# jskvrna/MonoSOWA

Hardware: AMD Instinct MI355X
Metric: MonoDETR training img/s (KITTI 1280x384) (higher is better)
Workload: dtype f32; 1 GPU; MonoDETR resnet50 KITTI 1280x384, fwd+criterion+bwd+AdamW step, per-GPU batch 16, synthetic images + random pseudo-labels; global_batch=16, per_gpu_batch=16, parallelism=dp1, accumulation_micro_steps=1, mixed_cameras=False, queries=550, tuned=True

## Files before the change

monosowa_amd/build.py:

```python
import os
import shutil
import subprocess
import sys

HERE = os.path.dirname(os.path.abspath(__file__))
CSRC = os.path.join(HERE, "csrc")
LIBDIR = os.path.join(HERE, "lib")
ARCH = "gfx950"

LIBS = {
    "libmonosowa_msda.so": ("msda_capi.hip", []),
    "libmonosowa_pointwise.so": ("pointwise.hip", []),
    "libmonosowa_attn.so": ("flash_attn.hip", []),
    "libmonosowa_kitti.so": ("rotate_iou.hip", []),
    "libmonosowa_gemm.so": ("gemm_lt.cpp", ["-lhipblaslt"]),
    "libmonosowa_image.so": ("image_prep.hip", ["-ffp-contract=off"]),
    "libmonosowa_fit.so": ("template_fit.hip", []),
    "libmonosowa_lift.so": ("object_lift.hip", []),
    "libmonosowa_track.so": ("object_track.hip", []),
}

FLAGS = ["-O3", "--offload-arch=" + ARCH, "-munsafe-fp-atomics", "-fPIC", "-shared", "-std=c++17",
         "-fno-gpu-rdc", "-Wall"]


def hipcc():
    exe = shutil.which("hipcc") or "/opt/rocm/bin/hipcc"
    if not os.path.exists(exe):
        raise RuntimeError("hipcc not found: the MI355X-native kernels cannot be built")
    return exe


def source_hash(extra=()):
    import hashlib
    h = hashlib.sha256()
    inc = os.path.normpath(os.path.join(HERE, "..", "include"))
    files = [os.path.join(CSRC, f) for f in os.listdir(CSRC)] + [os.path.join(inc, f) for f in os.listdir(inc)]
    for path in sorted(files):
        if os.path.isfile(path):
            h.update(os.path.basename(path).encode() + b"\0")
            with open(path, "rb") as f:
                h.update(f.read())
            h.update(b"\0")
    for x in extra:
        h.update(str(x).encode() + b"\0")
    return h.hexdigest()


def _recorded_hash(out):
    try:
        with open(out + ".srchash") as f:
            return f.read().strip()
    except OSError:
        return None


def _build_one(out, cmd, want, force, verbose):
    name = os.path.basename(out)
    if not force and os.path.exists(out) and _recorded_hash(out) == want:
        if verbose:
            print("%s: up to date (source hash %s)" % (name, want[:16]), flush=True)
        return False
    if verbose:
        print(" ".join(cmd), flush=True)
    subprocess.check_call(cmd)
    with open(out + ".srchash", "w") as f:
        f.write(want + "\n")
    if verbose:
        print("%s: compiled (source hash %s)" % (name, want[:16]), flush=True)
    return True


def build_host_libs(force=False, verbose=False):
    out = os.path.join(LIBDIR, "libmonosowa_lsap.so")
    src = os.path.join(CSRC, "lsap.cpp")
    flags = ["-O3", "-fPIC", "-shared", "-std=c++17", "-Wall", "-pthread"]
    cmd = [shutil.which("g++") or "g++"] + flags + ["-o", out, src]
    _build_one(out, cmd, source_hash(["g++"] + flags), force, verbose)
    return [out]


def build_all(force=False, verbose=False):
    os.makedirs(LIBDIR, exist_ok=True)
    built = build_host_libs(force, verbose)
    for name, (tu, extra) in LIBS.items():
        out = os.path.join(LIBDIR, name)
        want = source_hash(["hipcc"] + FLAGS + extra)
        _build_one(out, [hipcc()] + FLAGS + ["-o", out, os.path.join(CSRC, tu)] + extra, want, force, verbose)
        built.append(out)
    _stamp_commit()
    return built


def _stamp_commit():
    try:
        root = os.path.dirname(HERE)
        h = subprocess.run(["git", "-C", root, "rev-parse", "--short", "HEAD"], capture_output=True, text=True, timeout=10)
        if h.returncode != 0:
            return
        d = subprocess.run(["git", "-C", root, "status", "--porcelain", "--untracked-files=no"], capture_output=True, text=True, timeout=10)
        with open(os.path.join(LIBDIR, "BUILD_COMMIT"), "w") as f:
            f.write(h.stdout.strip() + ("-dirty" if d.stdout.strip() else "") + "\n")
    except Exception:
        pass


if __name__ == "__main__":
    for p in build_all(force="--force" in sys.argv, verbose=True):
        print("built", p)
```

monosowa_amd/monodetr/backbone.py:

```python
import os

import torch
import torch.nn.functional as F
from torch import nn

from ..pointwise import (affine_relu, affine_relu_supported, bias_act, bias_act_fork, bias_relu_maxpool,
                         bias_relu_maxpool_supported, conv1x1_head, conv1x1_head_supported, conv1x1_tail,
                         conv1x1_tail_ds, conv1x1_tail_ds_supported, conv1x1_tail_supported)
from .misc import NestedTensor
from .position_encoding import build_position_encoding


AFFINE_IN_KERNEL = True
CACHE_SCALE_SHIFT = True


class FrozenBatchNorm2d(nn.Module):

    def __init__(self, n, eps=1e-5):
        super().__init__()
        self.register_buffer("weight", torch.ones(n))
        self.register_buffer("bias", torch.zeros(n))
        self.register_buffer("running_mean", torch.zeros(n))
        self.register_buffer("running_var", torch.ones(n))
        self.eps = eps

    def _load_from_state_dict(self, state_dict, prefix, local_metadata, strict, missing_keys,
                              unexpected_keys, error_msgs):
        state_dict.pop(prefix + "num_batches_tracked", None)
        super()._load_from_state_dict(state_dict, prefix, local_metadata, strict, missing_keys,
                                      unexpected_keys, error_msgs)

    def scale_shift(self):
        bufs = (self.weight, self.bias, self.running_mean, self.running_var)
        key = tuple((b.data_ptr(), b._version, b.device, b.dtype) for b in bufs)
        cached = self.__dict__.get("_scale_shift")
        if CACHE_SCALE_SHIFT and cached is not None and cached[0] == key:
            return cached[1], cached[2]
        scale = self.weight * (self.running_var + self.eps).rsqrt()
        shift = self.bias - self.running_mean * scale
        self.__dict__["_scale_shift"] = (key, scale, shift)
        return scale, shift

    def forward(self, x):
        scale, shift = self.scale_shift()
        return x * scale.reshape(1, -1, 1, 1) + shift.reshape(1, -1, 1, 1)


_PARAM_EPOCH = [0]


def _bump_param_epoch(*_args, **_kwargs):
    _PARAM_EPOCH[0] += 1


try:
    from torch.optim.optimizer import register_optimizer_step_post_hook
    register_optimizer_step_post_hook(_bump_param_epoch)
except ImportError:
    _PARAM_EPOCH = None


def folded_weight(conv, bn, scale):
    w = conv.weight
    if (w.requires_grad and torch.is_grad_enabled()) or _PARAM_EPOCH is None:
        return w * scale.view(-1, 1, 1, 1)
    key = (w.data_ptr(), w._version, scale.data_ptr(), scale._version, _PARAM_EPOCH[0] if w.requires_grad else -1)
    cached = conv.__dict__.get("_folded")
    if cached is None or cached[0] != key:
        with torch.no_grad():
            cached = conv.__dict__["_folded"] = (key, (w * scale.view(-1, 1, 1, 1)).contiguous(memory_format=torch.channels_last)
                                                 if w.is_contiguous(memory_format=torch.channels_last) else w * scale.view(-1, 1, 1, 1))
    return cached[1]


def _summed_shift(bn, other):
    a, b = bn.scale_shift()[1], other.scale_shift()[1]
    key = (a.data_ptr(), a._version, b.data_ptr(), b._version)
    cached = bn.__dict__.get("_summed_shift")
    if cached is None or cached[0] != key:
        with torch.no_grad():
            cached = bn.__dict__["_summed_shift"] = (key, a + b)
    return cached[1]


CONV1X1_EPILOGUE = int(os.environ.get("MONOSOWA_CONV1X1_EPILOGUE", "3"))
CONV1X1_SCALED_GRAD = 1


def _pixels(t):
    return t.permute(0, 2, 3, 1).reshape(-1, t.shape[1])


class _Conv1x1BnAct(torch.autograd.Function):

    @staticmethod
    def forward(ctx, x, w, scale, shift, residual, n_out):
        from .. import gemm_lt
        N, C, H, W = x.shape
        K = w.shape[0]
        y = torch.empty((N, K, H, W), dtype=torch.float32, device=x.device, memory_format=torch.channels_last)
        gemm_lt.gemm_nt(_pixels(x), w.reshape(K, C), scale, shift, None if residual is None else _pixels(residual), True, out=_pixels(y))
        ctx.save_for_backward(x, w, scale, y)
        ctx.has_res = residual is not None
        return (y,) + tuple(y.detach() for _ in range(n_out - 1))

    @staticmethod
    def backward(ctx, *grads):
        from .. import gemm_lt
        from ..pointwise import relu_grad_from_output
        x, w, scale, y = ctx.saved_tensors
        N, C, H, W = x.shape
        K = w.shape[0]
        given = [t for t in grads if t is not None]
        pre_scaled = bool(CONV1X1_SCALED_GRAD) and not ctx.has_res and len(given) == 1 and scale.data_ptr() % 16 == 0 and scale.is_contiguous()
        g = relu_grad_from_output(given, y, scale if pre_scaled else None)
        gx = gw = None
        w2 = w.reshape(K, C)
        if ctx.needs_input_grad[0]:
            ws = w2 if pre_scaled else w2 * scale.view(-1, 1)
            if CONV1X1_EPILOGUE & 2:
                gx = torch.empty_like(x)
                gemm_lt.gemm_nn(_pixels(g), ws, out=_pixels(gx))
            else:
                gx = torch.ops.aten.convolution_backward(g, x, ws.view(K, C, 1, 1), None, (1, 1), (0, 0), (1, 1), False, (0, 0), 1,
                                                         (True, False, False))[0]
        if ctx.needs_input_grad[1]:
            gw = torch.ops.aten.convolution_backward(g, x, w, None, (1, 1), (0, 0), (1, 1), False, (0, 0), 1, (False, True, False))[1]
            if not pre_scaled:
                gw = gw * scale.view(-1, 1, 1, 1)
        return gx, gw, None, None, (g if ctx.has_res else None), None


def conv1x1_no_grad(x, conv, scale, shift, residual, relu):
    if not (CONV1X1_EPILOGUE & 1) or conv.kernel_size != (1, 1) or conv.stride != (1, 1) or conv.groups != 1 or conv.padding != (0, 0) \
            or not x.is_cuda or x.dim() != 4 or x.dtype != torch.float32 or not x.is_contiguous(memory_format=torch.channels_last) \
            or x.shape[1] % 4 or conv.weight.shape[0] % 4 \
            or (torch.is_grad_enabled() and (x.requires_grad or conv.weight.requires_grad or (residual is not None and residual.requires_grad))) \
            or (residual is not None and not (residual.shape[1] == conv.weight.shape[0] and residual.dtype == torch.float32
                                              and residual.is_contiguous(memory_format=torch.channels_last))):
        return None
    from .. import gemm_lt
    N, C, H, W = x.shape
    K = conv.weight.shape[0]
    y = torch.empty((N, K, H, W), dtype=torch.float32, device=x.device, memory_format=torch.channels_last)
    with torch.no_grad():
        gemm_lt.gemm_nt(_pixels(x), conv.weight.reshape(K, C), scale, shift, None if residual is None else _pixels(residual), relu, out=_pixels(y))
    return y


def conv1x1_epilogue_applies(x, conv, residual=None):
    from .. import gemm_lt
    return bool(CONV1X1_EPILOGUE & 1) and conv.kernel_size == (1, 1) and conv.stride == (1, 1) and conv.groups == 1 and conv.padding == (0, 0) \
        and x.is_cuda and x.dim() == 4 and x.dtype == torch.float32 and torch.is_grad_enabled() and conv.weight.requires_grad \
        and x.is_contiguous(memory_format=torch.channels_last) and x.shape[1] % 4 == 0 and conv.weight.shape[0] % 4 == 0 \
        and (residual is None or (residual.shape[1] == conv.weight.shape[0] and residual.is_contiguous(memory_format=torch.channels_last)
                                  and residual.dtype == torch.float32))


def conv_bn_fork(x, conv, bn, residual, n_out=2, residual_bn=None):
    if isinstance(bn, FrozenBatchNorm2d):
        scale, shift = bn.scale_shift()
        if residual_bn is not None:
            shift = _summed_shift(bn, residual_bn)
        if conv1x1_epilogue_applies(x, conv, residual):
            return _Conv1x1BnAct.apply(x, conv.weight, scale, shift, residual, n_out)
        y = conv1x1_no_grad(x, conv, scale, shift, residual, True)
        if y is not None:
            return (y,) * n_out
        y = F.conv2d(x, folded_weight(conv, bn, scale), None, conv.stride, conv.padding, conv.dilation, conv.groups)
        return bias_act_fork(y, shift, residual, n_out)
    assert residual_bn is None
    out = conv_bn(x, conv, bn, residual)
    return (out,) * n_out


def conv_bn(x, conv, bn, residual=None, relu=True):
    if isinstance(bn, FrozenBatchNorm2d):
        scale, shift = bn.scale_shift()
        if relu and residual is None and conv1x1_epilogue_applies(x, conv):
            return _Conv1x1BnAct.apply(x, conv.weight, scale, shift, None, 1)[0]
        if AFFINE_IN_KERNEL and relu and residual is None and conv.weight.requires_grad and torch.is_grad_enabled() and x.is_cuda:
            y = F.conv2d(x, conv.weight, None, conv.stride, conv.padding, conv.dilation, conv.groups)
            if affine_relu_supported(y, scale):
                return affine_relu(y, scale, shift)
            return torch.relu(y * scale.view(1, -1, 1, 1) + shift.view(1, -1, 1, 1))
        y = conv1x1_no_grad(x, conv, scale, shift, residual, relu)
        if y is not None:
            return y
        y = F.conv2d(x, folded_weight(conv, bn, scale), None, conv.stride, conv.padding, conv.dilation, conv.groups)
        return bias_act(y, shift, residual, relu)
    y = bn(conv(x))
    if residual is not None:
        y = y + residual
    return F.relu(y, inplace=True) if relu else y


FOLD_DOWNSAMPLE_SHIFT = os.environ.get("MONOSOWA_FOLD_DS_SHIFT", "1") != "0"
FUSED_FROZEN_DS = os.environ.get("MONOSOWA_FUSED_FROZEN_DS", "1") != "0"
FUSED_FROZEN_TAIL = os.environ.get("MONOSOWA_FUSED_FROZEN_TAIL", "1") != "0"
FUSED_STEM = os.environ.get("MONOSOWA_FUSED_STEM", "1") != "0"


def stem(x, conv, bn):
    if isinstance(bn, FrozenBatchNorm2d):
        scale, shift = bn.scale_shift()
        w = folded_weight(conv, bn, scale)
        if not (w.requires_grad and torch.is_grad_enabled()):
            y = F.conv2d(x, w, None, conv.stride, conv.padding, conv.dilation, conv.groups)
            if FUSED_STEM and bias_relu_maxpool_supported(y, shift):
                return bias_relu_maxpool(y, shift)
            return F.max_pool2d(bias_act(y, shift, None, True), kernel_size=3, stride=2, padding=1)
    return F.max_pool2d(conv_bn(x, conv, bn), kernel_size=3, stride=2, padding=1)


class Bottleneck(nn.Module):
    expansion = 4

    def __init__(self, inplanes, planes, stride=1, downsample=None, dilation=1, norm_layer=FrozenBatchNorm2d):
        super().__init__()
        self.conv1 = nn.Conv2d(inplanes, planes, 1, bias=False)
        self.bn1 = norm_layer(planes)
        self.conv2 = nn.Conv2d(planes, planes, 3, stride=stride, padding=dilation, dilation=dilation, bias=False)
        self.bn2 = norm_layer(planes)
        self.conv3 = nn.Conv2d(planes, planes * self.expansion, 1, bias=False)
        self.bn3 = norm_layer(planes * self.expansion)
        self.downsample = downsample

    def forward(self, x):
        xa, xb = x if isinstance(x, tuple) else (x, x)
        n_out = getattr(self, "n_out", 2)
        whole = self._frozen_block(xa, xb, n_out) if FUSED_FROZEN_TAIL else None
        if whole is not None:
            return whole
        out = conv_bn(xa, self.conv1, self.bn1)
        out = conv_bn(out, self.conv2, self.bn2)
        if self.downsample is None:
            return conv_bn_fork(out, self.conv3, self.bn3, xb, n_out)
        ds_conv, ds_bn = self.downsample[0], self.downsample[1]
        if FOLD_DOWNSAMPLE_SHIFT and isinstance(ds_bn, FrozenBatchNorm2d) and isinstance(self.bn3, FrozenBatchNorm2d):
            identity = F.conv2d(xb, folded_weight(ds_conv, ds_bn, ds_bn.scale_shift()[0]), None, ds_conv.stride, ds_conv.padding,
                                ds_conv.dilation, ds_conv.groups)
            return conv_bn_fork(out, self.conv3, self.bn3, identity, n_out, residual_bn=ds_bn)
        identity = conv_bn(xb, ds_conv, ds_bn, relu=False)
        return conv_bn_fork(out, self.conv3, self.bn3, identity, n_out)


    def _frozen_block(self, xa, xb, n_out):
        bn1, bn2, bn3, ds = self.bn1, self.bn2, self.bn3, self.downsample
        if self.conv3.weight.shape[:2] != (256, 64) or not xa.is_cuda or not isinstance(bn2, FrozenBatchNorm2d) \
                or not isinstance(bn3, FrozenBatchNorm2d) or (ds is not None and not isinstance(ds[1], FrozenBatchNorm2d)):
            return None
        if torch.is_grad_enabled() and (xa.requires_grad or xb.requires_grad or self.conv1.weight.requires_grad
                                        or self.conv2.weight.requires_grad or self.conv3.weight.requires_grad
                                        or (ds is not None and ds[0].weight.requires_grad)):
            return None
        h1 = None
        conv1 = self.conv1
        if isinstance(bn1, FrozenBatchNorm2d) and conv1.kernel_size == (1, 1) and conv1.stride == (1, 1) and conv1.weight.shape[0] == 64:
            scale1, shift1 = bn1.scale_shift()
            w1 = folded_weight(conv1, bn1, scale1)
            cached = self.__dict__.get("_head_w")
            if cached is None or cached[0] is not w1:
                with torch.no_grad():
                    cached = self.__dict__["_head_w"] = (w1, w1.reshape(64, -1).t().contiguous())
            if conv1x1_head_supported(xa, cached[1]):
                h1 = conv1x1_head(xa, cached[1], shift1)
        if h1 is None:
            h1 = conv_bn(xa, conv1, bn1)
        (scale2, shift2), (scale3, shift3) = bn2.scale_shift(), bn3.scale_shift()
        w3 = folded_weight(self.conv3, bn3, scale3)
        cached = self.__dict__.get("_tail_w")
        if cached is None or cached[0] is not w3:
            with torch.no_grad():
                cached = self.__dict__["_tail_w"] = (w3, w3.reshape(256, 64).t().contiguous())
        w_kn = cached[1]
        conv2 = self.conv2
        raw2 = F.conv2d(h1, folded_weight(conv2, bn2, scale2), None, conv2.stride, conv2.padding, conv2.dilation, conv2.groups)
        if ds is not None and FUSED_FROZEN_DS and ds[0].kernel_size == (1, 1) and ds[0].stride == (1, 1) and ds[0].weight.shape[:2] == (256, 64):
            wd = folded_weight(ds[0], ds[1], ds[1].scale_shift()[0])
            cached_d = self.__dict__.get("_tail_wd")
            if cached_d is None or cached_d[0] is not wd:
                with torch.no_grad():
                    cached_d = self.__dict__["_tail_wd"] = (wd, wd.reshape(256, 64).t().contiguous())
            if conv1x1_tail_ds_supported(raw2, w_kn, xb, cached_d[1]):
                return (conv1x1_tail_ds(raw2, shift2, w_kn, xb, cached_d[1], _summed_shift(bn3, ds[1])),) * n_out
        if ds is None:
            identity, b_out = xb, shift3
        else:
            identity = F.conv2d(xb, folded_weight(ds[0], ds[1], ds[1].scale_shift()[0]), None, ds[0].stride, ds[0].padding,
                                ds[0].dilation, ds[0].groups)
            b_out = _summed_shift(bn3, ds[1])
        if not conv1x1_tail_supported(raw2, w_kn, identity):
            out = bias_act(raw2, shift2, None, True)
            y = F.conv2d(out, w3, None, self.conv3.stride, self.conv3.padding, self.conv3.dilation, self.conv3.groups)
            return (bias_act(y, b_out, identity, True),) * n_out
        return (conv1x1_tail(raw2, shift2, w_kn, b_out, identity),) * n_out


_DEPTHS = {"resnet50": (3, 4, 6, 3), "resnet101": (3, 4, 23, 3)}


class ResNetBody(nn.Module):

    def __init__(self, name, dilation=False, norm_layer=FrozenBatchNorm2d, return_interm_layers=True):
        super().__init__()
        if name not in _DEPTHS:
            raise ValueError("backbone %r is not supported (resnet50 / resnet101)" % name)
        self.inplanes, self._dil = 64, 1
        self.conv1 = nn.Conv2d(3, 64, 7, stride=2, padding=3, bias=False)
        self.bn1 = norm_layer(64)
        self.layer1 = self._make_layer(64, _DEPTHS[name][0], 1, False, norm_layer)
        self.layer2 = self._make_layer(128, _DEPTHS[name][1], 2, False, norm_layer)
        self.layer3 = self._make_layer(256, _DEPTHS[name][2], 2, False, norm_layer)
        self.layer4 = self._make_layer(512, _DEPTHS[name][3], 2, dilation, norm_layer)
        self.return_interm_layers = return_interm_layers
        for m in self.modules():
            if isinstance(m, nn.Conv2d):
                nn.init.kaiming_normal_(m.weight, mode="fan_out", nonlinearity="relu")

    def _make_layer(self, planes, blocks, stride, dilate, norm_layer):
        prev_dil = self._dil
        if dilate:
            self._dil *= stride
            stride = 1
        downsample = None
        if stride != 1 or self.inplanes != planes * 4:
            downsample = nn.Sequential(nn.Conv2d(self.inplanes, planes * 4, 1, stride=stride, bias=False),
                                       norm_layer(planes * 4))
        layers = [Bottleneck(self.inplanes, planes, stride, downsample, prev_dil, norm_layer)]
        self.inplanes = planes * 4
        layers += [Bottleneck(self.inplanes, planes, dilation=self._dil, norm_layer=norm_layer) for _ in range(1, blocks)]
        return nn.Sequential(*layers)

    def forward(self, x):
        x = stem(x, self.conv1, self.bn1)
        x = self.layer1(x)
        if self.return_interm_layers:
            self.layer2[-1].n_out = self.layer3[-1].n_out = 3
        c3 = self.layer2(x)
        c4 = self.layer3(c3[:2])
        c5 = self.layer4(c4[:2])
        out5 = c5[0]
        if c5[1] is not c5[0]:
            out5.fork_twin = c5[1]
        return {"0": c3[-1], "1": c4[-1], "2": out5} if self.return_interm_layers else {"0": out5}


class Backbone(nn.Module):

    def __init__(self, name, train_backbone, return_interm_layers, dilation, depth=False, pretrained=False):
        super().__init__()
        if depth:
            raise NotImplementedError("4-channel (RGB-D) input is off in every shipped config (model.depth: False)")
        if pretrained:
            raise RuntimeError("model.pretrained: True needs torchvision's ImageNet download, which is not "
                               "available offline; load a state dict instead and set pretrained: False")
        assert name not in ("resnet18", "resnet34"), "number of channels are hard coded"
        self.body = ResNetBody(name, dilation, FrozenBatchNorm2d, return_interm_layers)
        for pname, p in self.body.named_parameters():
            if not train_backbone or ("layer2" not in pname and "layer3" not in pname and "layer4" not in pname):
                p.requires_grad_(False)
        if return_interm_layers:
            self.strides, self.num_channels = [8, 16, 32], [512, 1024, 2048]
        else:
            self.strides, self.num_channels = [32], [2048]
        if dilation:
            self.strides[-1] = self.strides[-1] // 2

    def forward(self, images):
        out = {}
        for name, x in self.body(images).items():
            mask = torch.zeros(x.shape[0], x.shape[2], x.shape[3], dtype=torch.bool, device=x.device)
            out[name] = NestedTensor(x, mask, all_valid=True)
        return out


class Joiner(nn.Sequential):
    def __init__(self, backbone, position_embedding):
        super().__init__(backbone, position_embedding)
        self.strides = backbone.strides
        self.num_channels = backbone.num_channels

    def forward(self, images):
        xs = self[0](images)
        out = [x for _, x in sorted(xs.items())]
        pos = [self[1](x).to(x.tensors.dtype) for x in out]
# ... 10 lines not shown
```

monosowa_amd/pointwise.py:

```python
import ctypes
import os

import numpy as np
import torch

from . import flops
from ._lib import raw_stream, on_device, DeterministicSwitch, alert_not_deterministic

_PATH = os.path.join(os.path.dirname(os.path.abspath(__file__)), "lib", "libmonosowa_pointwise.so")
SYMBOLS = ("mono_bias_act_f32", "mono_bias_relu_maxpool_nhwc_f32", "mono_conv1x1_tail_f32", "mono_conv1x1_tail_ds_f32", "mono_conv1x1_head_f32", "mono_relu_grad_f32", "mono_relu_grad2_f32", "mono_relu_grad3_f32", "mono_bias_relu_mask_f32", "mono_relu_grad_mask_f32", "mono_affine_relu_mask_f32", "mono_affine_relu_grad_f32", "mono_dropout_add_layernorm_fwd_f32",
           "mono_dropout_add_layernorm_bwd_f32", "mono_groupnorm_nhwc_fwd_f32", "mono_groupnorm_nhwc_bwd_f32", "mono_groupnorm_blocks", "mono_colsum_f32", "mono_colsum_strided_f32", "mono_reduce_blocks", "mono_adamw_step_f32", "mono_adamw_step_guarded_f32", "mono_grad_guard_f32", "mono_relu_dropout_fwd_f32",
           "mono_relu_dropout_bwd_f32", "mono_matched_losses_fwd_f32", "mono_matched_losses_bwd_f32", "mono_ddn_loss_blocks",
           "mono_ddn_loss_fwd_f32", "mono_ddn_loss_bwd_f32", "mono_depth_expect_fwd_f32", "mono_depth_expect_bwd_f32", "mono_focal_fwd_f32", "mono_focal_bwd_f32", "mono_head_tail_fwd_f32", "mono_head_tail_bwd_f32", "mono_match_cost_f32", "mono_refine_reference_f32", "mono_relu_dropout_bwd_colsum_f32", "mono_sum_slices_f32", "mono_colsum_any_blocks", "mono_colsum_any_f32", "mono_relu_grad_mask3_f32", "mono_lsap_match_flat_f32",
           "mono_linear_wgrad_workspace", "mono_linear_wgrad_f32", "mono_colsum_levels_blocks", "mono_colsum_levels_f32", "mono_relu_grad_scale_f32",
           "mono_set_deterministic", "mono_groupnorm_stats_doubles", "mono_groupnorm_part_doubles", "mono_grad_accumulate_f32", "mono_ema_update_f32", "mono_step_stats_f32",
           "mono_label_audit_f32", "mono_matched_losses_weighted_fwd_f32", "mono_matched_losses_weighted_bwd_f32", "mono_focal_weighted_fwd_f32",
           "mono_focal_weighted_bwd_f32", "mono_ddn_loss_weighted_fwd_f32", "mono_ddn_loss_weighted_bwd_f32", "mono_focal_weighted_max_cells",
           "mono_ignore_flags_f32", "mono_focal_ignore_fwd_f32", "mono_focal_ignore_bwd_f32", "mono_focal_weighted_ignore_fwd_f32",
           "mono_focal_weighted_ignore_bwd_f32", "mono_ddn_loss_ignore_fwd_f32", "mono_ddn_loss_ignore_bwd_f32",
           "mono_ddn_loss_weighted_ignore_fwd_f32", "mono_ddn_loss_weighted_ignore_bwd_f32")
_lib = None


def load():
# ... 136 lines not shown
        lib.mono_ddn_loss_weighted_fwd_f32.restype = I
        lib.mono_ddn_loss_weighted_fwd_f32.argtypes = [P] * 6 + [I] * 5 + [LL] * 3 + [F] * 6 + [P]
        lib.mono_ddn_loss_weighted_bwd_f32.restype = I
        lib.mono_ddn_loss_weighted_bwd_f32.argtypes = [P] * 7 + [I] * 5 + [LL] * 3 + [F] * 6 + [P]
        for name, n_ptr in (("mono_ddn_loss_ignore_fwd_f32", 8), ("mono_ddn_loss_ignore_bwd_f32", 8), ("mono_ddn_loss_weighted_ignore_fwd_f32", 9),
                            ("mono_ddn_loss_weighted_ignore_bwd_f32", 9)):
            getattr(lib, name).restype = I
            getattr(lib, name).argtypes = [P] * n_ptr + [I] * 6 + [LL] * 3 + [F] * 6 + [P]
        _lib = lib
    return _lib


def _nhwc_ok(t):
    return t.is_cuda and t.dtype == torch.float32 and t.dim() == 4 and t.size(1) % 4 == 0 \
        and t.is_contiguous(memory_format=torch.channels_last) and t.data_ptr() % 16 == 0


USE_RELU_MASK = True


class _BiasAct(torch.autograd.Function):
    @staticmethod
    def forward(ctx, y, bias, residual, relu):
        rows = y.numel() // y.size(1)
        res_ptr = residual.data_ptr() if residual is not None else None
        mask = None
        with on_device(y.device):
            st = raw_stream()
            if relu and USE_RELU_MASK and (y.requires_grad or (residual is not None and residual.requires_grad)):
                mask = torch.empty(y.numel() // 4, dtype=torch.uint8, device=y.device)
                code = load().mono_bias_relu_mask_f32(y.data_ptr(), bias.data_ptr(), res_ptr, mask.data_ptr(), rows, y.size(1), st)
            else:
                code = load().mono_bias_act_f32(y.data_ptr(), bias.data_ptr(), res_ptr, rows, y.size(1), int(relu), st)
        if code:
            raise RuntimeError("mono_bias_act_f32 failed with code %d" % code)
        ctx.mark_dirty(y)
        ctx.relu = relu
        ctx.has_res = residual is not None
        ctx.bias_grad = bias.requires_grad
        ctx.masked = mask is not None
        if relu:
            ctx.save_for_backward(mask if mask is not None else y)
        return y

    @staticmethod
    def backward(ctx, grad):
        if ctx.relu:
            (y,) = ctx.saved_tensors
            grad = grad.contiguous(memory_format=torch.channels_last)
            g = torch.empty_like(grad, memory_format=torch.channels_last)
            with on_device(y.device):
                if ctx.masked:
                    code = load().mono_relu_grad_mask_f32(grad.data_ptr(), None, y.data_ptr(), g.data_ptr(), grad.numel(),
                                                          raw_stream())
                else:
                    code = load().mono_relu_grad_f32(grad.data_ptr(), y.data_ptr(), g.data_ptr(), grad.numel(),
                                                     raw_stream())
            if code:
                raise RuntimeError("mono_relu_grad_f32 failed with code %d" % code)
        else:
            g = grad
        gb = g.sum((0, 2, 3)) if ctx.bias_grad else None
        return g, gb, (g if ctx.has_res else None), None


class _AffineRelu(torch.autograd.Function):

    @staticmethod
    def forward(ctx, y, scale, shift):
        rows, C = y.numel() // y.size(1), y.size(1)
        mask = torch.empty(y.numel() // 4, dtype=torch.uint8, device=y.device)
        with on_device(y.device):
            code = load().mono_affine_relu_mask_f32(y.data_ptr(), scale.data_ptr(), shift.data_ptr(), mask.data_ptr(), rows, C,
                                                    raw_stream())
        if code:
            raise RuntimeError("mono_affine_relu_mask_f32 failed with code %d" % code)
        ctx.mark_dirty(y)
        ctx.save_for_backward(mask, scale)
        return y

    @staticmethod
    def backward(ctx, grad):
        mask, scale = ctx.saved_tensors
        grad = grad.contiguous(memory_format=torch.channels_last)
        g = torch.empty_like(grad, memory_format=torch.channels_last)
        with on_device(grad.device):
            code = load().mono_affine_relu_grad_f32(grad.data_ptr(), mask.data_ptr(), scale.data_ptr(), g.data_ptr(),
                                                    grad.numel() // grad.size(1), grad.size(1), raw_stream())
        if code:
            raise RuntimeError("mono_affine_relu_grad_f32 failed with code %d" % code)
        return g, None, None


def affine_relu_supported(y, scale):
    return _nhwc_ok(y) and y.requires_grad and torch.is_grad_enabled() and scale.is_cuda and scale.dtype == torch.float32 \
        and scale.data_ptr() % 16 == 0 and not scale.requires_grad


def affine_relu(y, scale, shift):
    return _AffineRelu.apply(y, scale.contiguous(), shift.contiguous())


class _BiasActFork(torch.autograd.Function):

    @staticmethod
    def forward(ctx, y, bias, residual, n_out=2):
        rows = y.numel() // y.size(1)
        mask = torch.empty(y.numel() // 4, dtype=torch.uint8, device=y.device) if USE_RELU_MASK else None
        with on_device(y.device):
            st = raw_stream()
            if mask is not None:
                code = load().mono_bias_relu_mask_f32(y.data_ptr(), bias.data_ptr(), residual.data_ptr(), mask.data_ptr(), rows, y.size(1), st)
            else:
                code = load().mono_bias_act_f32(y.data_ptr(), bias.data_ptr(), residual.data_ptr(), rows, y.size(1), 1, st)
        if code:
            raise RuntimeError("mono_bias_act_f32 failed with code %d" % code)
        ctx.mark_dirty(y)
        ctx.save_for_backward(mask if mask is not None else y)
        ctx.masked = mask is not None
        ctx.shape = y.shape
        ctx.bias_grad = bias.requires_grad
        return (y, y.detach()) if n_out == 2 else (y, y.detach(), y.detach())

    @staticmethod
    def backward(ctx, ga, gb, gc=None):
        (y,) = ctx.saved_tensors
        cl = lambda t: t.contiguous(memory_format=torch.channels_last)
        lib = load()
        g = torch.empty(ctx.shape, dtype=torch.float32, device=y.device, memory_format=torch.channels_last)
        n = g.numel()
        given = [cl(t) for t in (ga, gb, gc) if t is not None]
        if len(given) == 3 and not ctx.masked:
            given = [given[0] + given[1], given[2]]
        with on_device(y.device):
            st = raw_stream()
            if len(given) == 3:
                code = lib.mono_relu_grad_mask3_f32(given[0].data_ptr(), given[1].data_ptr(), given[2].data_ptr(), y.data_ptr(), g.data_ptr(), n, st)
            elif len(given) == 2:
                if ctx.masked:
                    code = lib.mono_relu_grad_mask_f32(given[0].data_ptr(), given[1].data_ptr(), y.data_ptr(), g.data_ptr(), n, st)
                else:
                    code = lib.mono_relu_grad2_f32(given[0].data_ptr(), given[1].data_ptr(), y.data_ptr(), g.data_ptr(), n, st)
            else:
                if ctx.masked:
                    code = lib.mono_relu_grad_mask_f32(given[0].data_ptr(), None, y.data_ptr(), g.data_ptr(), n, st)
                else:
                    code = lib.mono_relu_grad_f32(given[0].data_ptr(), y.data_ptr(), g.data_ptr(), n, st)
        if code:
            raise RuntimeError("mono_relu_grad(2)_f32 failed with code %d" % code)
        return g, (g.sum((0, 2, 3)) if ctx.bias_grad else None), g, None


def relu_grad_from_output(grads, y, scale=None):
    cl = lambda t: t.contiguous(memory_format=torch.channels_last)
    given = [cl(t) for t in grads]
    g = torch.empty(y.shape, dtype=torch.float32, device=y.device, memory_format=torch.channels_last)
    n = g.numel()
    lib = load()
    if scale is not None and len(given) != 1:
        raise ValueError("relu_grad_from_output: a scale goes with exactly one gradient")
    with on_device(y.device):
        if scale is not None:
            code = lib.mono_relu_grad_scale_f32(given[0].data_ptr(), y.data_ptr(), scale.data_ptr(), g.data_ptr(), n, y.shape[1], raw_stream())
        elif len(given) == 3:
            code = lib.mono_relu_grad3_f32(given[0].data_ptr(), given[1].data_ptr(), given[2].data_ptr(), y.data_ptr(), g.data_ptr(), n, raw_stream())
        elif len(given) == 2:
            code = lib.mono_relu_grad2_f32(given[0].data_ptr(), given[1].data_ptr(), y.data_ptr(), g.data_ptr(), n, raw_stream())
        else:
            code = lib.mono_relu_grad_f32(given[0].data_ptr(), y.data_ptr(), g.data_ptr(), n, raw_stream())
    if code:
        raise RuntimeError("mono_relu_grad(2)_f32 failed with code %d" % code)
    return g


def bias_relu_maxpool_supported(y, bias):
    return _nhwc_ok(y) and bias.is_cuda and bias.dtype == torch.float32 and bias.data_ptr() % 16 == 0 and bias.numel() == y.size(1) \
        and not (torch.is_grad_enabled() and (y.requires_grad or bias.requires_grad))


def bias_relu_maxpool(y, bias):
    N, C, H, W = y.shape
    out = torch.empty((N, C, (H - 1) // 2 + 1, (W - 1) // 2 + 1), dtype=torch.float32, device=y.device, memory_format=torch.channels_last)
    with on_device(y.device):
        code = load().mono_bias_relu_maxpool_nhwc_f32(y.data_ptr(), bias.data_ptr(), out.data_ptr(), N, H, W, C, raw_stream())
    if code:
        raise RuntimeError("mono_bias_relu_maxpool_nhwc_f32 failed with code %d" % code)
    return out


def conv1x1_tail_supported(x, w_kn, residual):
    return _nhwc_ok(x) and _nhwc_ok(residual) and x.size(1) == 64 and residual.size(1) == 256 and tuple(w_kn.shape) == (64, 256) \
        and x.shape[0] == residual.shape[0] and x.shape[2:] == residual.shape[2:] and w_kn.is_contiguous() and w_kn.data_ptr() % 16 == 0 \
        and not (torch.is_grad_enabled() and (x.requires_grad or residual.requires_grad or w_kn.requires_grad))


def conv1x1_tail(x, b_in, w_kn, b_out, residual):
    out = torch.empty_like(residual)
    M = x.numel() // 64
    flops.conv1x1(M, 64, 256)
    with on_device(x.device):
        code = load().mono_conv1x1_tail_f32(x.data_ptr(), b_in.data_ptr(), w_kn.data_ptr(), b_out.data_ptr(), residual.data_ptr(),
                                            out.data_ptr(), M, 64, 256, raw_stream())
    if code:
        raise RuntimeError("mono_conv1x1_tail_f32 failed with code %d" % code)
    return out


def conv1x1_tail_ds_supported(x, w_kn, x0, wd_kn):
    ok_w = lambda w: tuple(w.shape) == (64, 256) and w.is_contiguous() and w.data_ptr() % 16 == 0 and not (torch.is_grad_enabled() and w.requires_grad)
    return _nhwc_ok(x) and _nhwc_ok(x0) and x.size(1) == 64 and x0.shape == x.shape and ok_w(w_kn) and ok_w(wd_kn) \
        and not (torch.is_grad_enabled() and (x.requires_grad or x0.requires_grad))


def conv1x1_tail_ds(x, b_in, w_kn, x0, wd_kn, b_out):
    N, _, H, W = x.shape
    out = torch.empty((N, 256, H, W), dtype=torch.float32, device=x.device, memory_format=torch.channels_last)
    flops.conv1x1(N * H * W, 128, 256)
    with on_device(x.device):
        code = load().mono_conv1x1_tail_ds_f32(x.data_ptr(), b_in.data_ptr(), w_kn.data_ptr(), x0.data_ptr(), wd_kn.data_ptr(), b_out.data_ptr(),
                                               out.data_ptr(), N * H * W, 64, 256, raw_stream())
    if code:
        raise RuntimeError("mono_conv1x1_tail_ds_f32 failed with code %d" % code)
    return out


def conv1x1_head_supported(x, w_kn):
    return _nhwc_ok(x) and x.size(1) in (64, 256) and tuple(w_kn.shape) == (x.size(1), 64) and w_kn.is_contiguous() \
        and w_kn.data_ptr() % 16 == 0 and not (torch.is_grad_enabled() and (x.requires_grad or w_kn.requires_grad))


def conv1x1_head(x, w_kn, b_out):
    N, K, H, W = x.shape
    out = torch.empty((N, 64, H, W), dtype=torch.float32, device=x.device, memory_format=torch.channels_last)
    flops.conv1x1(N * H * W, K, 64)
    with on_device(x.device):
        code = load().mono_conv1x1_head_f32(x.data_ptr(), w_kn.data_ptr(), b_out.data_ptr(), out.data_ptr(), N * H * W, K, 64, raw_stream())
    if code:
        raise RuntimeError("mono_conv1x1_head_f32 failed with code %d" % code)
    return out


def bias_act_fork(y, bias, residual, n_out=2):
    if _nhwc_ok(y) and bias.is_cuda and bias.dtype == torch.float32 and bias.data_ptr() % 16 == 0 \
            and _nhwc_ok(residual) and residual.shape == y.shape and torch.is_grad_enabled() and y.requires_grad:
        return _BiasActFork.apply(y, bias.contiguous(), residual, n_out)
    out = bias_act(y, bias, residual, True)
    return (out,) * n_out


def bias_act(y, bias, residual=None, relu=True):
    if _nhwc_ok(y) and bias.is_cuda and bias.dtype == torch.float32 and bias.data_ptr() % 16 == 0 \
            and (residual is None or (_nhwc_ok(residual) and residual.shape == y.shape)):
        return _BiasAct.apply(y, bias.contiguous(), residual, relu)
    out = y + bias.view(1, -1, 1, 1)
    if residual is not None:
        out = out + residual
    return torch.relu(out) if relu else out


_seed_counter = [0]


def _next_seed():
    _seed_counter[0] += 1
    rank = torch.distributed.get_rank() if torch.distributed.is_available() and torch.distributed.is_initialized() else 0
    return (torch.initial_seed() * 0x9E3779B97F4A7C15 + _seed_counter[0] * 0xD1B54A32D192ED03 + rank * 0x94D049BB133111EB) & (2 ** 64 - 1)


LN_MIN_ROWS = int(os.environ.get('MONOSOWA_LN_MIN_ROWS', '1'))


def row_dense(t):
    if t.is_contiguous():
        return True
    if t.dim() < 2 or t.stride(-1) != 1:
        return False
    order = sorted(range(t.dim() - 1), key=lambda d: -t.stride(d))
    return t.permute(*order, t.dim() - 1).is_contiguous()


def same_layout(ref, t):
    if t.stride() == ref.stride():
        return t
    return torch.empty_like(ref).copy_(t)


def ln_forward(x, z, weight, bias, p, eps):
    if not row_dense(x):
        x = x.contiguous()
    z = same_layout(x, z)
    rows = x.numel() // 256
    y, s = torch.empty_like(x), torch.empty_like(x)
    mean = torch.empty(rows, dtype=torch.float32, device=x.device)
    rstd = torch.empty_like(mean)
    seed = _next_seed() if p > 0 else 0
    with on_device(x.device):
        code = load().mono_dropout_add_layernorm_fwd_f32(
            x.data_ptr(), z.data_ptr(), weight.data_ptr(), bias.data_ptr(), y.data_ptr(), s.data_ptr(), mean.data_ptr(),
            rstd.data_ptr(), rows, 256, float(p), seed, float(eps), raw_stream())
    if code:
        raise RuntimeError("mono_dropout_add_layernorm_fwd_f32 failed with code %d" % code)
    return y, s, mean, rstd, seed


def ln_backward(gy, s, mean, rstd, weight, p, seed, with_gz_sum=False):
    gy = same_layout(s, gy)
# ... 1164 lines not shown
```

Before: 245.8 img/s.

## Fuse ResNet identity bottleneck backward with CK GEMM relu-mask epilogues

Adds a Composable Kernel GEMM with multiple-D epilogues that computes the data gradient and applies the ReLU mask, optionally with a per-channel scale or a residual add. A new autograd function handles the whole identity bottleneck block. It uses these epilogues for the conv3 and conv1 data-gradient GEMMs, and it lets the next block pass an already-masked gradient back so the producer skips its relu_grad pass. The aim is to remove separate elementwise passes and extra activation-sized reads and writes in the backbone backward. The trade-offs are fixed CK tile instances that may run slower than hipBLASLt, and fragile graph inspection to detect the premask case.

```diff
diff --git a/include/monosowa_gemm_epi.h b/include/monosowa_gemm_epi.h
--- /dev/null
+++ b/include/monosowa_gemm_epi.h
@@ -0,0 +1,26 @@
+#ifndef MONOSOWA_GEMM_EPI_H
+#define MONOSOWA_GEMM_EPI_H
+
+#ifdef __cplusplus
+extern "C" {
+#endif
+
+#define MONO_GEMM_EPI_E_NULLPTR (-1)
+#define MONO_GEMM_EPI_E_NOT_SERVED (-4)
+
+int mono_gemm_nn_add_relumask_f32(const float *A, long long lda, const float *B, long long ldb, const float *D, long long ldd,
+                                  const float *Y, long long ldy, float *E, long long lde, int M, int N, int K, void *stream);
+
+int mono_gemm_nn_scale_relumask_f32(const float *A, long long lda, const float *B, long long ldb, const float *s, const float *Y,
+                                    long long ldy, float *E, long long lde, int M, int N, int K, void *stream);
+
+int mono_gemm_epi_served(int M, int N, int K, long long lda, long long ldb, long long ldmn);
+
+int mono_gemm_epi_instances(void);
+int mono_gemm_epi_table(int N, int K);
+int mono_gemm_epi_force_instance(int index);
+
+#ifdef __cplusplus
+}
+#endif
+#endif
diff --git a/monosowa_amd/build.py b/monosowa_amd/build.py
--- a/monosowa_amd/build.py
+++ b/monosowa_amd/build.py
@@ -14,6 +14,7 @@
     "libmonosowa_attn.so": ("flash_attn.hip", []),
     "libmonosowa_kitti.so": ("rotate_iou.hip", []),
     "libmonosowa_gemm.so": ("gemm_lt.cpp", ["-lhipblaslt"]),
+    "libmonosowa_gemm_epi.so": ("gemm_epilogue.hip", []),
     "libmonosowa_image.so": ("image_prep.hip", ["-ffp-contract=off"]),
     "libmonosowa_fit.so": ("template_fit.hip", []),
     "libmonosowa_lift.so": ("object_lift.hip", []),
diff --git a/monosowa_amd/csrc/gemm_epilogue.hip b/monosowa_amd/csrc/gemm_epilogue.hip
--- /dev/null
+++ b/monosowa_amd/csrc/gemm_epilogue.hip
@@ -0,0 +1,133 @@
+#include <hip/hip_runtime.h>
+
+#include <array>
+#include <atomic>
+#include <cstdint>
+
+#include "ck/ck.hpp"
+#include "ck/tensor_operation/gpu/device/gemm_specialization.hpp"
+#include "ck/tensor_operation/gpu/device/impl/device_gemm_multiple_d_xdl_cshuffle.hpp"
+#include "ck/tensor_operation/gpu/device/tensor_layout.hpp"
+#include "ck/tensor_operation/gpu/element/element_wise_operation.hpp"
+
+#include "../../include/monosowa_gemm_epi.h"
+
+namespace mono {
+
+__host__ __device__ inline bool relu_on_hd(float v) { return !(v <= 0.f); }
+
+struct AddReluMask {
+  template <typename E, typename C, typename D0, typename D1>
+  __host__ __device__ constexpr void operator()(E &e, const C &c, const D0 &d, const D1 &y) const {
+    e = relu_on_hd(y) ? c + d : 0.f;
+  }
+};
+
+struct ScaleReluMask {
+  template <typename E, typename C, typename D0, typename D1>
+  __host__ __device__ constexpr void operator()(E &e, const C &c, const D0 &s, const D1 &y) const {
+    e = relu_on_hd(y) ? c * s : 0.f;
+  }
+};
+
+using F32 = float;
+using Row = ck::tensor_layout::gemm::RowMajor;
+using Pass = ck::tensor_operation::element_wise::PassThrough;
+template <ck::index_t... Is>
+using S = ck::Sequence<Is...>;
+
+template <typename Op, int MPerBlock, int NPerBlock, int KPerBlock, int MXdl, int NXdl, typename AClu, typename BClu, int BVec>
+using Gemm = ck::tensor_operation::device::DeviceGemmMultipleD_Xdl_CShuffle<
+    Row, Row, ck::Tuple<Row, Row>, Row, F32, F32, F32, F32, ck::Tuple<F32, F32>, F32, Pass, Pass, Op,
+    ck::tensor_operation::device::GemmSpecialization::Default, 1, 256, MPerBlock, NPerBlock, KPerBlock, 4, 4, 32, 32, MXdl, NXdl,
+    AClu, S<1, 0, 2>, S<1, 0, 2>, 2, 4, 4, 1,
+    BClu, S<0, 2, 1>, S<0, 2, 1>, 1, BVec, 4, 1,
+    1, 1, S<1, 16, 1, 16>, 4>;
+
+struct Tile { int m, n, k; };
+constexpr int kInstances = 2;
+constexpr Tile kTiles[kInstances] = {{256, 128, 16}, {128, 128, 16}};
+
+template <typename Op> using Inst0 = Gemm<Op, 256, 128, 16, 4, 2, S<4, 64, 1>, S<4, 64, 1>, 2>;
+template <typename Op> using Inst1 = Gemm<Op, 128, 128, 16, 2, 2, S<4, 64, 1>, S<4, 64, 1>, 2>;
+
+std::atomic<int> g_forced{-1};
+
+int table(int N, int K) {
+  (void)N;
+  (void)K;
+  return 1;
+}
+
+int pick(int N, int K) {
+  const int f = g_forced.load();
+  return (f >= 0 && f < kInstances) ? f : table(N, K);
+}
+
+bool tiles_fit(int i, int M, int N, int K) { return M % kTiles[i].m == 0 && N % kTiles[i].n == 0 && K % kTiles[i].k == 0; }
+
+bool operand_ok(const void *p, long long rows, long long cols, long long ld) {
+  if (((uintptr_t)p & 15) || (ld & 3) || (ld != 0 && ld < cols)) return false;
+  const long long bytes = ((rows - 1) * ld + cols) * 4;
+  return bytes < (1ll << 31);
+}
+
+template <typename G, typename Op>
+int run(const float *A, long long lda, const float *B, long long ldb, const float *D0, long long ld0, const float *D1, long long ld1,
+        float *E, long long lde, int M, int N, int K, hipStream_t stream) {
+  try {
+    auto arg = G::MakeArgument(A, B, std::array<const void *, 2>{D0, D1}, E, M, N, K, (ck::index_t)lda, (ck::index_t)ldb,
+                               std::array<ck::index_t, 2>{(ck::index_t)ld0, (ck::index_t)ld1}, (ck::index_t)lde, Pass{}, Pass{},
+                               Op{});
+    if (!G::IsSupportedArgument(arg)) return MONO_GEMM_EPI_E_NOT_SERVED;
+    G::MakeInvoker().Run(arg, StreamConfig{stream, false});
+  } catch (...) {
+    return MONO_GEMM_EPI_E_NOT_SERVED;
+  }
+  return (int)hipGetLastError();
+}
+
+template <typename Op>
+int dispatch(const float *A, long long lda, const float *B, long long ldb, const float *D0, long long ld0, const float *D1, long long ld1,
+             float *E, long long lde, int M, int N, int K, void *stream_) {
+  if (!operand_ok(A, M, K, lda) || !operand_ok(B, K, N, ldb) || !operand_ok(D0, M, N, ld0) || !operand_ok(D1, M, N, ld1) ||
+      !operand_ok(E, M, N, lde) || lde == 0)
+    return MONO_GEMM_EPI_E_NOT_SERVED;
+  const int i = pick(N, K);
+  if (!tiles_fit(i, M, N, K)) return MONO_GEMM_EPI_E_NOT_SERVED;
+  hipStream_t st = (hipStream_t)stream_;
+  switch (i) {
+    case 0: return run<Inst0<Op>, Op>(A, lda, B, ldb, D0, ld0, D1, ld1, E, lde, M, N, K, st);
+    default: return run<Inst1<Op>, Op>(A, lda, B, ldb, D0, ld0, D1, ld1, E, lde, M, N, K, st);
+  }
+}
+
+}
+
+extern "C" {
+
+int mono_gemm_nn_add_relumask_f32(const float *A, long long lda, const float *B, long long ldb, const float *D, long long ldd,
+                                  const float *Y, long long ldy, float *E, long long lde, int M, int N, int K, void *stream) {
+  if (!A || !B || !D || !Y || !E || M <= 0 || N <= 0 || K <= 0 || lda <= 0 || ldb <= 0 || ldd <= 0 || ldy <= 0 || lde <= 0)
+    return MONO_GEMM_EPI_E_NULLPTR;
+  return mono::dispatch<mono::AddReluMask>(A, lda, B, ldb, D, ldd, Y, ldy, E, lde, M, N, K, stream);
+}
+
+int mono_gemm_nn_scale_relumask_f32(const float *A, long long lda, const float *B, long long ldb, const float *s, const float *Y,
+                                    long long ldy, float *E, long long lde, int M, int N, int K, void *stream) {
+  if (!A || !B || !s || !Y || !E || M <= 0 || N <= 0 || K <= 0 || lda <= 0 || ldb <= 0 || ldy <= 0 || lde <= 0)
+    return MONO_GEMM_EPI_E_NULLPTR;
+  return mono::dispatch<mono::ScaleReluMask>(A, lda, B, ldb, s, 0, Y, ldy, E, lde, M, N, K, stream);
+}
+
+int mono_gemm_epi_served(int M, int N, int K, long long lda, long long ldb, long long ldmn) {
+  if (M <= 0 || N <= 0 || K <= 0 || lda <= 0 || ldb <= 0 || ldmn <= 0) return MONO_GEMM_EPI_E_NULLPTR;
+  if (!mono::operand_ok(nullptr, M, K, lda) || !mono::operand_ok(nullptr, K, N, ldb) || !mono::operand_ok(nullptr, M, N, ldmn)) return 0;
+  return mono::tiles_fit(mono::pick(N, K), M, N, K) ? 1 : 0;
+}
+
+int mono_gemm_epi_instances(void) { return mono::kInstances; }
+int mono_gemm_epi_table(int N, int K) { return (N > 0 && K > 0) ? mono::table(N, K) : MONO_GEMM_EPI_E_NULLPTR; }
+int mono_gemm_epi_force_instance(int index) { return mono::g_forced.exchange(index < mono::kInstances ? index : -1); }
+
+}
diff --git a/monosowa_amd/gemm_epi.py b/monosowa_amd/gemm_epi.py
--- /dev/null
+++ b/monosowa_amd/gemm_epi.py
@@ -0,0 +1,101 @@
+import ctypes
+import os
+
+import torch
+
+from ._lib import on_device, raw_stream
+
+_PATH = os.path.join(os.path.dirname(os.path.abspath(__file__)), "lib", "libmonosowa_gemm_epi.so")
+SYMBOLS = ("mono_gemm_nn_add_relumask_f32", "mono_gemm_nn_scale_relumask_f32", "mono_gemm_epi_served", "mono_gemm_epi_instances",
+           "mono_gemm_epi_table", "mono_gemm_epi_force_instance")
+E_NULLPTR, E_NOT_SERVED = -1, -4
+_lib = None
+
+CALLS = {"add": 0, "scale": 0, "add_pair": 0, "scale_pair": 0}
+
+
+def reset_calls():
+    for k in CALLS:
+        CALLS[k] = 0
+
+
+def load():
+    global _lib
+    if _lib is None:
+        if not os.path.exists(_PATH):
+            raise RuntimeError("HIP extension %s is missing: run `python -m monosowa_amd.build`" % _PATH)
+        lib = ctypes.CDLL(_PATH)
+        P, I, L = ctypes.c_void_p, ctypes.c_int, ctypes.c_longlong
+        lib.mono_gemm_nn_add_relumask_f32.restype = I
+        lib.mono_gemm_nn_add_relumask_f32.argtypes = [P, L, P, L, P, L, P, L, P, L, I, I, I, P]
+        lib.mono_gemm_nn_scale_relumask_f32.restype = I
+        lib.mono_gemm_nn_scale_relumask_f32.argtypes = [P, L, P, L, P, P, L, P, L, I, I, I, P]
+        lib.mono_gemm_epi_served.restype = I
+        lib.mono_gemm_epi_served.argtypes = [I, I, I, L, L, L]
+        lib.mono_gemm_epi_instances.restype = I
+        lib.mono_gemm_epi_table.restype = I
+        lib.mono_gemm_epi_table.argtypes = [I, I]
+        lib.mono_gemm_epi_force_instance.restype = I
+        lib.mono_gemm_epi_force_instance.argtypes = [I]
+        _lib = lib
+    return _lib
+
+
+def served(M, N, K, lda=None, ldb=None, ldmn=None):
+    return load().mono_gemm_epi_served(M, N, K, K if lda is None else lda, N if ldb is None else ldb, N if ldmn is None else ldmn) == 1
+
+
+def _mat(t):
+    return t.is_cuda and t.dtype == torch.float32 and t.dim() == 2 and t.stride(1) == 1
+
+
+def add_relumask(a, b, d, y, out=None, fallback=True):
+    M, K = a.shape
+    N = b.shape[1]
+    assert b.shape[0] == K and d.shape == (M, N) and y.shape == (M, N) and all(_mat(t) for t in (a, b, d, y))
+    if out is None:
+        out = torch.empty((M, N), dtype=torch.float32, device=a.device)
+    with on_device(a.device):
+        code = load().mono_gemm_nn_add_relumask_f32(a.data_ptr(), a.stride(0), b.data_ptr(), b.stride(0), d.data_ptr(), d.stride(0),
+                                                    y.data_ptr(), y.stride(0), out.data_ptr(), out.stride(0), M, N, K, raw_stream())
+    if code == 0:
+        CALLS["add"] += 1
+        return out, True
+    if code != E_NOT_SERVED:
+        raise RuntimeError("mono_gemm_nn_add_relumask_f32 failed with code %d" % code)
+    if not fallback:
+        return None, False
+    from . import gemm_lt, pointwise
+    prod = gemm_lt.gemm_nn(a, b)
+    with on_device(a.device):
+        if out.is_contiguous() and d.is_contiguous() and y.is_contiguous() and out.numel() % 4 == 0:
+            code = pointwise.load().mono_relu_grad2_f32(prod.data_ptr(), d.data_ptr(), y.data_ptr(), out.data_ptr(), out.numel(), raw_stream())
+            if code:
+                raise RuntimeError("mono_relu_grad2_f32 failed with code %d" % code)
+        else:
+            torch.where(y <= 0, torch.zeros((), device=a.device), prod + d, out=out)
+    CALLS["add_pair"] += 1
+    return out, False
+
+
+def scale_relumask(a, b, s, y, out=None, fallback=True):
+    M, K = a.shape
+    N = b.shape[1]
+    assert b.shape[0] == K and s.shape == (N,) and s.is_contiguous() and y.shape == (M, N) and all(_mat(t) for t in (a, b, y))
+    if out is None:
+        out = torch.empty((M, N), dtype=torch.float32, device=a.device)
+    with on_device(a.device):
+        code = load().mono_gemm_nn_scale_relumask_f32(a.data_ptr(), a.stride(0), b.data_ptr(), b.stride(0), s.data_ptr(), y.data_ptr(),
+                                                      y.stride(0), out.data_ptr(), out.stride(0), M, N, K, raw_stream())
+    if code == 0:
+        CALLS["scale"] += 1
+        return out, True
+    if code != E_NOT_SERVED:
+        raise RuntimeError("mono_gemm_nn_scale_relumask_f32 failed with code %d" % code)
+    if not fallback:
+        return None, False
+    from . import gemm_lt
+    prod = gemm_lt.gemm_nn(a, b)
+    torch.where(y <= 0, torch.zeros((), device=a.device), prod * s, out=out)
+    CALLS["scale_pair"] += 1
+    return out, False
diff --git a/monosowa_amd/monodetr/backbone.py b/monosowa_amd/monodetr/backbone.py
--- a/monosowa_amd/monodetr/backbone.py
+++ b/monosowa_amd/monodetr/backbone.py
@@ -84,7 +84,9 @@
     return cached[1]
 
 
-CONV1X1_EPILOGUE = int(os.environ.get("MONOSOWA_CONV1X1_EPILOGUE", "3"))
+_EPILOGUE_BITS = int(os.environ.get("MONOSOWA_CONV1X1_EPILOGUE", "7"))
+CONV1X1_EPILOGUE = _EPILOGUE_BITS & 3
+CONV1X1_DX_EPILOGUE = _EPILOGUE_BITS & 12
 CONV1X1_SCALED_GRAD = 1
 
 
@@ -103,6 +105,8 @@
         gemm_lt.gemm_nt(_pixels(x), w.reshape(K, C), scale, shift, None if residual is None else _pixels(residual), True, out=_pixels(y))
         ctx.save_for_backward(x, w, scale, y)
         ctx.has_res = residual is not None
+        ctx.n_out = n_out
+        ctx.set_materialize_grads(False)
         return (y,) + tuple(y.detach() for _ in range(n_out - 1))
 
     @staticmethod
@@ -114,7 +118,10 @@
         K = w.shape[0]
         given = [t for t in grads if t is not None]
         pre_scaled = bool(CONV1X1_SCALED_GRAD) and not ctx.has_res and len(given) == 1 and scale.data_ptr() % 16 == 0 and scale.is_contiguous()
-        g = relu_grad_from_output(given, y, scale if pre_scaled else None)
+        if ctx.has_res and _premasked(ctx, grads):
+            g = grads[0]
+        else:
+            g = relu_grad_from_output(given, y, scale if pre_scaled else None)
         gx = gw = None
         w2 = w.reshape(K, C)
         if ctx.needs_input_grad[0]:
@@ -130,6 +137,102 @@
             if not pre_scaled:
                 gw = gw * scale.view(-1, 1, 1, 1)
         return gx, gw, None, None, (g if ctx.has_res else None), None
+
+
+def _premasked(ctx, grads):
+    return getattr(ctx, "premasked", False) and grads[0] is not None and all(t is None for t in grads[1:]) \
+        and grads[0].is_contiguous(memory_format=torch.channels_last)
+
+
+class _IdentityBottleneck(torch.autograd.Function):
+
+    @staticmethod
+    def forward(ctx, x, w1, w2, w3, scale1, shift1, scale2, shift2, scale3, shift3, padding, dilation, n_out, premask):
+        from .. import gemm_lt
+        from ..pointwise import load as pointwise_lib
+        from .._lib import on_device, raw_stream
+        N, C, H, W = x.shape
+        P = w1.shape[0]
+        y1 = torch.empty((N, P, H, W), dtype=torch.float32, device=x.device, memory_format=torch.channels_last)
+        gemm_lt.gemm_nt(_pixels(x), w1.reshape(P, C), scale1, shift1, None, True, out=_pixels(y1))
+        y2 = F.conv2d(y1, w2, None, (1, 1), padding, dilation, 1)
+        if not y2.is_contiguous(memory_format=torch.channels_last):
+            y2 = y2.contiguous(memory_format=torch.channels_last)
+        mask2 = torch.empty(y2.numel() // 4, dtype=torch.uint8, device=x.device)
+        with on_device(x.device):
+            code = pointwise_lib().mono_affine_relu_mask_f32(y2.data_ptr(), scale2.data_ptr(), shift2.data_ptr(), mask2.data_ptr(),
+                                                             N * H * W, P, raw_stream())
+        if code:
+            raise RuntimeError("mono_affine_relu_mask_f32 failed with code %d" % code)
+        y3 = torch.empty((N, C, H, W), dtype=torch.float32, device=x.device, memory_format=torch.channels_last)
+        gemm_lt.gemm_nt(_pixels(y2), w3.reshape(C, P), scale3, shift3, _pixels(x), True, out=_pixels(y3))
+        ctx.save_for_backward(x, w1, w2, w3, scale1, scale2, scale3, y1, y2, mask2, y3)
+        ctx.padding, ctx.dilation, ctx.n_out, ctx.premask = padding, dilation, n_out, premask
+        ctx.set_materialize_grads(False)
+        return (y3,) + tuple(y3.detach() for _ in range(n_out - 1))
+
+    @staticmethod
+    def backward(ctx, *grads):
+        from .. import gemm_epi, gemm_lt
+        from ..pointwise import load as pointwise_lib, relu_grad_from_output
+        from .._lib import on_device, raw_stream
+        x, w1, w2, w3, scale1, scale2, scale3, y1, y2, mask2, y3 = ctx.saved_tensors
+        N, C, H, W = x.shape
+        P = w1.shape[0]
+        M = N * H * W
+        wgrad = lambda g, inp, w: torch.ops.aten.convolution_backward(g, inp, w, None, (1, 1), (0, 0), (1, 1), False, (0, 0), 1,
+                                                                      (False, True, False))[1]
+        g = grads[0] if _premasked(ctx, grads) else relu_grad_from_output([t for t in grads if t is not None], y3)
+        ws3 = w3.reshape(C, P) * scale3.view(-1, 1)
+        g2 = torch.empty_like(y2)
+        if not (CONV1X1_DX_EPILOGUE & 8 and gemm_epi.scale_relumask(_pixels(g), ws3, scale2, _pixels(y2), out=_pixels(g2), fallback=False)[1]):
+            gx2 = torch.empty_like(y2)
+            gemm_lt.gemm_nn(_pixels(g), ws3, out=_pixels(gx2))
+            with on_device(x.device):
+                code = pointwise_lib().mono_affine_relu_grad_f32(gx2.data_ptr(), mask2.data_ptr(), scale2.data_ptr(), g2.data_ptr(), M, P,
+                                                                 raw_stream())
+            if code:
+                raise RuntimeError("mono_affine_relu_grad_f32 failed with code %d" % code)
+        gw3 = wgrad(g, y2, w3) * scale3.view(-1, 1, 1, 1)
+        gx1, gw2, _ = torch.ops.aten.convolution_backward(g2, y1, w2, None, (1, 1), ctx.padding, ctx.dilation, False, (0, 0), 1,
+                                                          (True, True, False))
+        g1 = relu_grad_from_output([gx1], y1, scale1)
+        gx = torch.empty_like(x)
+        if ctx.premask:
+            gemm_epi.add_relumask(_pixels(g1), w1.reshape(P, C), _pixels(g), _pixels(x), out=_pixels(gx))
+        else:
+            gemm_lt.gemm_nn(_pixels(g1), w1.reshape(P, C), out=_pixels(gx))
+            gx.add_(g)
+        gw1 = wgrad(g1, x, w1)
+        return (gx, gw1, gw2, gw3) + (None,) * 10
+
+
+def _identity_block_applies(blk, xa, xb):
+    if not (CONV1X1_DX_EPILOGUE & 4) or (CONV1X1_EPILOGUE & 3) != 3 or not AFFINE_IN_KERNEL or not CONV1X1_SCALED_GRAD or blk.downsample is not None \
+            or not torch.is_grad_enabled() or not xa.requires_grad:
+        return None
+    fn = xa.grad_fn
+    if xb is xa:
+        mode = "plain"
+    elif fn is not None and xb.grad_fn is fn and type(fn) in (_Conv1x1BnAct._backward_cls, _IdentityBottleneck._backward_cls) \
+            and getattr(fn, "n_out", 0) == 2 and getattr(fn, "has_res", True) and (xa.output_nr, xb.output_nr) == (0, 1) \
+            and xa.data_ptr() == xb.data_ptr():
+        mode = "premask"
+    else:
+        return None
+    c1, c2, c3 = blk.conv1, blk.conv2, blk.conv3
+    if not all(isinstance(b, FrozenBatchNorm2d) for b in (blk.bn1, blk.bn2, blk.bn3)) \
+            or not all(c.weight.requires_grad and c.weight.dtype == torch.float32 for c in (c1, c2, c3)) \
+            or not conv1x1_epilogue_applies(xa, c1) or c3.kernel_size != (1, 1) or c3.stride != (1, 1) or c3.padding != (0, 0) \
+            or c3.groups != 1 or c3.weight.shape[0] != xa.shape[1] or c3.weight.shape[1] % 4 \
+            or c2.stride != (1, 1) or c2.groups != 1 or c2.padding_mode != "zeros":
+        return None
+    for bn in (blk.bn1, blk.bn2, blk.bn3):
+        if any(not (t.is_cuda and t.dtype == torch.float32 and t.is_contiguous() and t.data_ptr() % 16 == 0) for t in bn.scale_shift()):
+            return None
+    from .. import gemm_epi
+    N, C, H, W = xa.shape
+    return mode if gemm_epi.served(N * H * W, C, c1.weight.shape[0]) else None
 
 
 def conv1x1_no_grad(x, conv, scale, shift, residual, relu):
@@ -233,6 +336,13 @@
         whole = self._frozen_block(xa, xb, n_out) if FUSED_FROZEN_TAIL else None
         if whole is not None:
             return whole
+        mode = _identity_block_applies(self, xa, xb) if self.downsample is None else None
+        if mode is not None:
+            if mode == "premask":
+                xa.grad_fn.premasked = True
+            (s1, b1), (s2, b2), (s3, b3) = self.bn1.scale_shift(), self.bn2.scale_shift(), self.bn3.scale_shift()
+            return _IdentityBottleneck.apply(xa, self.conv1.weight, self.conv2.weight, self.conv3.weight, s1, b1, s2, b2, s3, b3,
+                                             self.conv2.padding, self.conv2.dilation, n_out, mode == "premask")
         out = conv_bn(xa, self.conv1, self.bn1)
         out = conv_bn(out, self.conv2, self.bn2)
         if self.downsample is None:
diff --git a/monosowa_amd/pointwise.py b/monosowa_amd/pointwise.py
--- a/monosowa_amd/pointwise.py
+++ b/monosowa_amd/pointwise.py
@@ -312,6 +312,8 @@
 
 
 def relu_grad_from_output(grads, y, scale=None):
+    if not 1 <= len(grads) <= 3:
+        raise ValueError("relu_grad_from_output: 1 - 3 gradients, got %d" % len(grads))
     cl = lambda t: t.contiguous(memory_format=torch.channels_last)
     given = [cl(t) for t in grads]
     g = torch.empty(y.shape, dtype=torch.float32, device=y.device, memory_format=torch.channels_last)
```

Measured after the change: 248.4 img/s, median of 4. Within noise of the previous version (+1.1%).
